# EmbersArc/SCpp

Hardware: AMD Instinct MI355X
Metric: converged SCvx trajectories/sec (RocketQuat, K=50) at 1/2/4/8 MI355X (higher is better)
Workload: dtype f64

## Files before the change

### scpp_amd/csrc/common.h

```cpp
#pragma once
#ifdef SCPP_HIP_EMU
#include "hip_emu.h"
#else
#include <hip/hip_runtime.h>
typedef double d4_t __attribute__((ext_vector_type(4)));
#endif
#include <cmath>
#include <cstdint>

namespace scpp
{

constexpr int WAVE = 64;

#ifdef SCPP_HIP_EMU
#define WAVE_SYNC() __syncthreads()
#else
#define WAVE_SYNC()                                            \
    do                                                         \
    {                                                          \
        __builtin_amdgcn_fence(__ATOMIC_ACQ_REL, "wavefront"); \
        __builtin_amdgcn_wave_barrier();                       \
    } while (0)
#endif

#ifdef SCPP_HIP_EMU
template <class T>
inline T *uniformPtr(T *p) { return p; }
inline int uniformInt(int v) { return v; }
#else
template <class T>
__device__ __forceinline__ T *uniformPtr(T *p)
{
    const unsigned long long v = reinterpret_cast<unsigned long long>(p);
    const unsigned lo = __builtin_amdgcn_readfirstlane(unsigned(v)), hi = __builtin_amdgcn_readfirstlane(unsigned(v >> 32));
    typedef __attribute__((address_space(1))) T *gptr_t;
    return (T *)(gptr_t)((unsigned long long)(hi) << 32 | lo);
}
__device__ __forceinline__ int uniformInt(int v) { return __builtin_amdgcn_readfirstlane(v); }
#endif

#ifdef SCPP_HIP_EMU
inline double fastRcp(double d) { return 1. / d; }
inline double fastRsqrt(double d) { return 1. / sqrt(d); }
#else
__device__ __forceinline__ double fastRcp(double d)
{
    double r = __builtin_amdgcn_rcp(d);
    double e = __builtin_fma(-d, r, 1.);
    r = __builtin_fma(r, e, r);
    e = __builtin_fma(-d, r, 1.);
    r = __builtin_fma(r, e, r);
    return r;
}
__device__ __forceinline__ double fastRsqrt(double d)
{
    double y = __builtin_amdgcn_rsq(d);
    double h = 0.5 * y, e = __builtin_fma(-d * y, h, 0.5);
    y = __builtin_fma(y, e, y);
    h = 0.5 * y;
    e = __builtin_fma(-d * y, h, 0.5);
    y = __builtin_fma(y, e, y);
// ... 208 lines not shown
```

### scpp_amd/csrc/ipm_kernel.h

```cpp
#pragma once
#include "common.h"
#include "cone_math.h"
#include "constraint_table.h"
#include <type_traits>
#include <utility>

namespace scpp
{
namespace ipm
{

#ifndef IPM_FAC_ALIGN
#define IPM_FAC_ALIGN 1
#endif
template <class P>
struct Lay : Derived<P>
{
    using D = Derived<P>;
    static constexpr int NX = P::NX, NU = P::NU, NXV = P::NXV, NUV = P::NUV, NS = D::NS, NL = D::NL, HS_N = D::HS_N;
    static constexpr int F_W = 0;
    static constexpr int F_DL = F_W + NV;
    static constexpr int F_DW = F_DL + 1;
    static constexpr int F_DDL = F_DW + NV;
    static constexpr int F_WBAR = F_DDL + 1;
// ... 161 lines not shown
    double feastol, abstol, reltol, gamma;
    int maxit;
    int use_mfma;
};

#ifdef SCPP_HIP_EMU
#define LDSP
#else
#define LDSP __attribute__((address_space(3)))
#endif
enum SegLdsSlot
{
    SL_LAM = 0,
    SL_NU,
    SL_NUB,
    NSEGLDS
};
struct Ctx
{
    LDSP double *segl;
    int K, lane;
    int pitch;
    int setup_v0;
    double *st;
    double *sg;
    double *dy;
    double *fac;
    double *sv;
    double *sx;
    double *gsave;
    const double *A, *B, *C, *S, *Z;
    const double *ip;
};

template <class P>
__host__ __device__ inline unsigned segLdsBytes(int K)
{
    return SegInLds<P>::value ? unsigned(NSEGLDS * Lay<P>::NL * recPitch(K) * 8) : 0u;
}

template <class F, int... Is>
__device__ inline void sforImpl(F &&f, std::integer_sequence<int, Is...>)
{
    (f(std::integral_constant<int, Is>{}), ...);
}
template <int N, class F>
// ... 311 lines not shown
```

### scpp_amd/csrc/ipm_solve.h

```cpp
#pragma once
#include "ipm_kernel.h"
#include "sweeps.h"
#include <type_traits>

namespace scpp
{
namespace ipm
{

#define IPM_BLOWN 1e30
#ifndef IPM_SPLIT_STEPS
#define IPM_SPLIT_STEPS 1
#endif
#ifndef IPM_FUSE_UPDATE
#define IPM_FUSE_UPDATE 1
#endif
#define IPM_NEG_GAP 1e-6
__device__ inline bool ipmGapBroken(double gap) { return fabs(gap) > IPM_BLOWN || gap < -IPM_NEG_GAP; }

struct Glob
{
    double sig, dsg, n1, sigbar;
    double ss, zs, s3, z3, sc3[3], zc3[3];
    double dsig, ddsg, dn1, dss, dzs, ds3, dz3, dsc3[3], dzc3[3];
    double seta, sw[3];
    double hsig, Hsd, Hdd, schur;
    double lamC[3], dsC[3], dzC[3];
};

struct KernelArgs
{
    int B, K;
    double *X, *U, *sigma;
    const double *A, *Bm, *C, *S, *Z;
    const double *ip;
    const double *uhat;
    double *ws;
    double *wtrx;
    int *active;
    int *converged, *sc_iters, *ipm_iters, *status;
    double *norm1_nu, *sum_delta, *delta_sigma;
    double nu_tol, delta_tol;
    int max_sc_iterations;
    int *warm;
    int do_sc_update;
    int setup_schedule;
    const int *dd_fresh;
    double *Xold, *Uold;
    Settings opt;
    double *dbg;
};

struct Rhs
{
    double s, ds, n1, rhs3;
};

__device__ inline double dLP(bool identity, double sv, double zv) { return identity ? 1. : zv / sv; }

template <class P>
__device__ inline void prepareFactor(const Ctx &c, bool identity, Glob &g)
{
    using L = Lay<P>;
    const int k = c.lane, K = c.K;
    if (k < K - 1 && identity)
    {
        const SV sg = makeSV(c.sg, (G_NFIELDS * L::NL), unsigned(k), c.pitch);
        const SV xs = makeSX(c.sx, L::XREC, K, unsigned(k));
#pragma unroll
// ... 1689 lines not shown
            inj_m = -1;
            if (sscanf(e, "%d:%lf:%lf:%lf", &inj_n, &inj_v[0], &inj_v[1], &inj_v[2]) != 4)
                inj_n = -1;
        }
    }
    const int call = inj_n >= 0 ? calls[lane & (LANES - 1)]++ : -1;
    if (inj_n >= 0 && (call == inj_n || call == inj_m))
    {
        pres = inj_v[0];
        dres = inj_v[1];
        gap = inj_v[2];
    }
}
#endif
struct ResAcc
{
    double gap, rx, ry, rz, xx, yy, zz, ss, rxs, sumnb;
};
struct PendingStep
{
    double om, sigmu, z3_old, dz3, dsig, alpha, alpha_d;
};
template <class P, int I0, int N, bool UPD>
__device__ inline void resSegChunk(const SV &sg, const SegLds &sl, const SV &dyz, const SV &xs, const SV &xsz, double z3, ResAcc &p, const PendingStep &u)
{
    using L = Lay<P>;
    double nu[N], nub[N], s1[N], z1[N], s2[N], z2[N], lam[N], S[N];
    ldf<N>(sg, G_S1 * L::NL + I0, s1);
    ldf<N>(sg, G_Z1 * L::NL + I0, z1);
    ldf<N>(sg, G_S2 * L::NL + I0, s2);
    ldf<N>(sg, G_Z2 * L::NL + I0, z2);
    ldl<P, SL_NU, I0, N>(sl, nu);
    ldl<P, SL_NUB, I0, N>(sl, nub);
    ldl<P, SL_LAM, I0, N>(sl, lam);
    ldf<N>(dyz, L::DY_S + I0, S);
    if constexpr (UPD)
    {
        double vl[N], bcl[N], p1[N], p2[N];
        ldf<N>(xs, L::X_VL + I0, vl);
        ldf<N>(xsz, L::X_BCL + I0, bcl);
        ldf<N>(sg, G_DS1 * L::NL + I0, p1);
        ldf<N>(sg, G_DS2 * L::NL + I0, p2);
        LOADS_ISSUED();
#pragma unroll
        for (int i = 0; i < N; i++)
        {
            const SegRhsRow r = segRhsRow<1>(nu[i], nub[i], s1[i], z1[i], s2[i], z2[i], lam[i], p1[i], p2[i], u.om, u.sigmu, u.z3_old, u.dz3);
// ... 14 lines not shown
        stf<N>(sg, G_S2 * L::NL + I0, s2);
        stf<N>(sg, G_Z2 * L::NL + I0, z2);
    }
    else
        LOADS_ISSUED();
#pragma unroll
    for (int i = 0; i < N; i++)
    {
        const double r1 = s1[i] - (nub[i] - nu[i]);
        const double r2 = s2[i] - (nub[i] + nu[i]);
        const double rnu = -lam[i] + z1[i] - z2[i];
        const double rnub = -z1[i] - z2[i] + z3;
        p.sumnb += nub[i];
        p.gap += s1[i] * z1[i] + s2[i] * z2[i];
        p.rz += r1 * r1 + r2 * r2;
        p.zz += z1[i] * z1[i] + z2[i] * z2[i];
        p.ss += s1[i] * s1[i] + s2[i] * s2[i];
        p.yy += lam[i] * lam[i];
        p.rx += rnu * rnu + rnub * rnub;
        p.xx += nu[i] * nu[i] + nub[i] * nub[i];
        p.rxs += S[i] * lam[i];
    }
}
template <class P, bool UPD>
PHASE_FN void phResiduals(const PRIV Ctx *cin, PRIV Glob *gp, PRIV Iter *ip_)
{
    EMU_PHASE(UPD ? "phResiduals<update>" : "phResiduals");
    using L = Lay<P>;
    constexpr int NX = P::NX, NU = P::NU;
    const Ctx c = uniformCtx(cin);
    const Views v = makeViews<P>(c);
    const int k = v.k;
    const SV &st = v.st, &stN = v.stN, &sg = v.sg, &sgP = v.sgP, &dy = v.dy, &dyP = v.dyP;
    const double *ip = c.ip;
    const unsigned fm = v.fm;
    PendingStep u{0., 0., 0., 0., 0., 0., 0.};
    if constexpr (UPD)
    {
        Glob g = loadPriv(gp);
        const double sigma_c = ip_->sigma_c;
        u.alpha = ip_->alpha;
        u.alpha_d = ip_->alpha_d;
        u.om = 1. - sigma_c;
        u.sigmu = sigma_c * double(ip_->mu);
        u.z3_old = g.z3;
        u.dz3 = g.dz3;
        u.dsig = g.dsig;
        const double alpha = u.alpha, alpha_d = u.alpha_d;
// ... 188 lines not shown
        {
            const bool fx = fm & (1u << j);
            const double r = -gw[j] + (fx ? 0. : acc[j]);
            rxw[j] = r;
            p.rx += fx ? 0. : r * r;
            p.xx += fx ? 0. : x0[j] * x0[j];
        }
        st[L::F_RXD] = rxd;
        stf<NV>(st, L::F_RXW, rxw);
        if (v.vsg)
            stf<L::NL>(sg, G_RY * L::NL, resv);
    }
    p.gap = waveSumDpp(p.gap);
    p.rx = waveSumDpp(p.rx);
    p.ry = waveSumDpp(p.ry);
    p.rz = waveSumDpp(p.rz);
    p.xx = waveSumDpp(p.xx);
    p.yy = waveSumDpp(p.yy);
    p.zz = waveSumDpp(p.zz);
    p.ss = waveSumDpp(p.ss);
    p.rxs = waveSumDpp(p.rxs);
    p.sumnb = waveSumDpp(p.sumnb);
    p_dl = waveSumDpp(p_dl);
    const Glob g = reloadPriv(gp);
    Iter it = reloadPriv(ip_);
    const double pres_before = it.pres;
    const double sas = g.sig - 0.001, sa3 = g.n1 - p.sumnb;
    const double sac[3] = {0.5 + 0.5 * g.dsg, 0.5 - 0.5 * g.dsg, g.sig - g.sigbar};
    it.rzs = g.ss - sas;
    it.rz3 = g.s3 - sa3;
    for (int i = 0; i < 3; i++)
        it.rzc[i] = g.sc3[i] - sac[i];
    it.rxs = it.w_t - g.zs - g.zc3[2] - p.rxs;
    it.rxds = it.w_trt - 0.5 * g.zc3[0] + 0.5 * g.zc3[1];
    it.rxn1 = it.w_vc - g.z3;
    double gap = p.gap + g.ss * g.zs + g.s3 * g.z3;
    double nrz = p.rz + it.rzs * it.rzs + it.rz3 * it.rz3;
    double nzz = p.zz + g.zs * g.zs + g.z3 * g.z3;
    double nss = p.ss + g.ss * g.ss + g.s3 * g.s3;
    for (int i = 0; i < 3; i++)
    {
        gap += g.sc3[i] * g.zc3[i];
        nrz += it.rzc[i] * it.rzc[i];
        nzz += g.zc3[i] * g.zc3[i];
        nss += g.sc3[i] * g.sc3[i];
    }
    const double nrx = p.rx + it.rxs * it.rxs + it.rxds * it.rxds + it.rxn1 * it.rxn1;
    const double nxx = p.xx + g.sig * g.sig + g.dsg * g.dsg + g.n1 * g.n1;
    it.gap = gap;
    it.mu = gap / it.D;
    it.pcost = it.w_t * g.sig + it.w_trt * g.dsg + it.w_vc * g.n1 + it.wtrx * p_dl;
    {
        const double nx_ = sqrt(nxx), ny_ = sqrt(p.yy), nz_ = sqrt(nzz), ns_ = sqrt(nss);
        const double d1 = it.resy0 + nx_ > 1. ? it.resy0 + nx_ : 1.;
        const double d2 = it.resz0 + nx_ + ns_ > 1. ? it.resz0 + nx_ + ns_ : 1.;
        const double pa = sqrt(p.ry) / d1, pb = sqrt(nrz) / d2;
        it.pres = pa > pb ? pa : pb;
        const double d3 = it.resx0 + ny_ + nz_ > 1. ? it.resx0 + ny_ + nz_ : 1.;
        it.dres = sqrt(nrx) / d3;
    }
#ifdef SCPP_HIP_EMU
    emuInjectResiduals(c.lane, it.pres, it.dres, it.gap);
#endif
    {
        const double apc = fabs(it.pcost) > 1e-300 ? fabs(it.pcost) : 1e-300;
        const bool broken = !(it.pres == it.pres) || !(it.dres == it.dres) || !(it.gap == it.gap) || fabs(it.pres) > 1e300 || fabs(it.dres) > 1e300 ||
                            ipmGapBroken(it.gap) || fabs(it.pcost) > IPM_BLOWN ||
                            (it.bk_valid != 0 && (it.pres > 500. * pres_before || it.gap < 0.));
        const bool inacc = !broken && it.pres < 1e-4 && it.dres < 1e-4 && (it.gap < 5e-5 || it.gap / apc < 5e-5);
        if (inacc)
        {
            if (v.vst)
            {
                double xw[NV + 1];
                ldf<NV + 1>(st, L::F_W, xw);
                stf<NV + 1>(st, L::F_WBK, xw);
            }
            it.bk_sig = g.sig;
            it.bk_dsg = g.dsg;
            it.bk_n1 = g.n1;
            it.bk_valid = 1;
        }
        PUT_BEGIN();
        PUT(ip_, it, rzs);
        PUT(ip_, it, rz3);
        PUT(ip_, it, rzc);
        PUT(ip_, it, rxs);
        PUT(ip_, it, rxds);
        PUT(ip_, it, rxn1);
        PUT(ip_, it, gap);
        PUT(ip_, it, mu);
        PUT(ip_, it, pcost);
        PUT(ip_, it, pres);
        PUT(ip_, it, dres);
        if (inacc)
        {
            PUT(ip_, it, bk_sig);
            PUT(ip_, it, bk_dsg);
            PUT(ip_, it, bk_n1);
            PUT(ip_, it, bk_valid);
        }
        PUT_END();
    }
}

template <class P>
PHASE_FN void phScalings(const PRIV Ctx *cin, PRIV Glob *gp, PRIV Iter *ip_)
{
    EMU_PHASE("phScalings");
    using L = Lay<P>;
    const Ctx c = uniformCtx(cin);
    const Views v = makeViews<P>(c);
    const SV &st = v.st;
    const unsigned act = v.act;
    const bool scvx = scvxMode(c.ip);
    const SV stz = padView(v.st, scvx);
    Glob g = loadPriv(gp);
    int bad = 0;
    if (v.vst)
    {
        forEachCone<P>([&](auto ci) {
            constexpr int C = decltype(ci)::value;
            if (act & (1u << C))
                bad |= coneScaling<P, L::coneOff(C), L::coneDim(C)>(st, C, stz);
        });
    }
// ... 723 lines not shown
        for (int i = 0; i < 10; i++)
            sh.prof[i] = 0.;
#endif
    const int K = a.K, lane = threadIdx.x, k = lane;
    Ctx c;
    c.K = K;
    c.lane = lane;
    double *ws = a.ws + size_t(inst) * workspaceDoubles<P>(K);
    c.sx = ws;
    c.st = ws + size_t(K) * L::XREC;
    c.pitch = recPitch(K);
    c.sg = c.st + size_t(c.pitch) * L::STREC;
    c.dy = c.sg + size_t(c.pitch) * (G_NFIELDS * L::NL);
    c.fac = ws + facOffset<P>(K);
    c.sv = c.fac + size_t(K) * L::FACREC;
    c.gsave = c.sv + size_t(K) * SVREC;
    c.A = a.A + size_t(inst) * (K - 1) * NX * NX;
    c.B = a.Bm + size_t(inst) * (K - 1) * NX * NU;
    c.C = a.C + size_t(inst) * (K - 1) * NX * NU;
    c.S = a.S + size_t(inst) * (K - 1) * NX;
    c.Z = a.Z + size_t(inst) * (K - 1) * NX;
    c.ip = a.ip + size_t(inst) * IP_N;
    c.setup_v0 = a.setup_schedule == 0;
    EMU_PHASE("solve: outside the phases");
    EMU_TRAFFIC_REGION("exchange [K][XREC]", c.sx, size_t(K) * L::XREC * 8, 8, size_t(L::XREC) * 8);
    EMU_TRAFFIC_REGION("stage [STREC][K]", c.st, size_t(c.pitch) * L::STREC * 8, size_t(c.pitch) * 8, 0);
    EMU_TRAFFIC_REGION("segment [G_NFIELDS*NL][K]", c.sg, size_t(c.pitch) * (G_NFIELDS * L::NL) * 8, size_t(c.pitch) * 8, 0);
    EMU_TRAFFIC_REGION("dd copy [DYNREC][K]", c.dy, size_t(c.pitch) * L::DYNREC * 8, size_t(c.pitch) * 8, 0);
    EMU_TRAFFIC_REGION("factor [K][FACREC]", c.fac, size_t(K) * L::FACREC * 8, 8, size_t(L::FACREC) * 8);
    EMU_TRAFFIC_REGION("saved columns [K][SVREC]", c.sv, size_t(K) * SVREC * 8, 8, size_t(SVREC) * 8);
    EMU_TRAFFIC_REGION("dd A [K-1][NX][NX]", c.A, size_t(K - 1) * NX * NX * 8, 8, size_t(NX) * NX * 8);
    EMU_TRAFFIC_REGION("dd B [K-1][NX][NU]", c.B, size_t(K - 1) * NX * NU * 8, 8, size_t(NX) * NU * 8);
    EMU_TRAFFIC_REGION("dd C [K-1][NX][NU]", c.C, size_t(K - 1) * NX * NU * 8, 8, size_t(NX) * NU * 8);
#ifdef SCPP_HIP_EMU
    static double seg_lds[NSEGLDS * 16 * 64];
    c.segl = seg_lds;
#else
    extern __shared__ __attribute__((aligned(16))) double seg_lds[];
    c.segl = (LDSP double *)seg_lds;
#endif
    const Settings opt = a.opt;

    __shared__ Glob g;
    __shared__ Iter it;
    __shared__ Ctx cshared;
    PRIV Glob *gp = (PRIV Glob *)&g;
// ... 45 lines not shown
            const RhsSpec sp = specSingle();
            fwdSweepAny<P>(cs, sp);
            bwdSweepAny<P>(cs, sp);
        }
        phInitDualFinish<P>(cs, gp, itp);
    }
    solveDataNorms<P>(cs, gp, itp, dd_same);
    phSegLdsCopy<P, true>(cs);
    PROF_T(tp1);
    PROF_ADD(0, tp0, tp1);

    status = -1;
    iter = 0;
    use_backup = false;
    it.bk_valid = 0;
    it.bad = 0;
    bool inacc_ok = false, bk_prev = false;
    double pres_prev = 0.;
    for (iter = 0;; iter++)
    {
        PROF_T(tr0);
#if IPM_FUSE_UPDATE
        if (iter == 0)
            phResiduals<P, false>(cs, gp, itp);
        else
            phResiduals<P, true>(cs, gp, itp);
#else
        phResiduals<P, false>(cs, gp, itp);
#endif
        PROF_T(tr1);
        PROF_ADD(1, tr0, tr1);
        {
            const double pres = it.pres, dres = it.dres, gap = it.gap;
            const double apc = fabs(it.pcost) > 1e-300 ? fabs(it.pcost) : 1e-300;
            const double relgap = gap / apc;
#ifdef SCPP_HIP_EMU
            if (c.lane == 0 && getenv("SCPP_EMU_DEBUG"))
                printf("[emu] iter %d pres %.3e dres %.3e gap %.3e pcost %.9e | last step: alpha %.3e alpha_d %.3e sigma_c %.3e\n", iter, pres, dres, gap, double(it.pcost),
                       double(it.alpha), double(it.alpha_d), double(it.sigma_c));
#endif
            const bool nonfinite = !(pres == pres) || !(dres == dres) || !(gap == gap) || fabs(pres) > 1e300 || fabs(dres) > 1e300 || fabs(gap) > 1e300 ||
                                   fabs(it.pcost) > IPM_BLOWN || ipmGapBroken(gap);
            if (nonfinite || (bk_prev && iter > 0 && (pres > 500. * pres_prev || gap < 0.)))
            {
                status = bk_prev ? 0 : -2;
                use_backup = bk_prev;
                break;
            }
            pres_prev = pres;
            bk_prev = it.bk_valid != 0;
            if (pres < opt.feastol && dres < opt.feastol && (gap < opt.abstol || relgap < opt.reltol))
// ... 188 lines not shown
```

### scpp_amd/csrc/ipm_split.h

```cpp
#pragma once
#include "ipm_solve.h"

namespace scpp
{
namespace ipm
{

#ifndef IPM_SPLIT_WAVES
#define IPM_SPLIT_WAVES 3
#endif

enum SplitPc
{
    PC_START = 0,
    PC_INIT_F = 1,
    PC_MAIN_F = 2,
    PC_NORMS = 3,
    PC_HEAD = 4,
    PC_END = 5,
    PC_DONE = 6
};
constexpr int RS_GLOB = 0, RS_ITER = RS_GLOB + int(sizeof(Glob) / 8), RS_LOC = RS_ITER + int(sizeof(Iter) / 8);
enum SplitLocal
{
// ... 17 lines not shown
    using L = Lay<P>;
    constexpr int NX = P::NX, NU = P::NU;
    const int K = a.K;
    Ctx c;
    c.K = K;
    c.lane = lane;
    double *ws = a.ws + size_t(inst) * workspaceDoubles<P>(K);
    c.sx = ws;
    c.st = ws + size_t(K) * L::XREC;
    c.pitch = recPitch(K);
    c.sg = c.st + size_t(c.pitch) * L::STREC;
    c.dy = c.sg + size_t(c.pitch) * (G_NFIELDS * L::NL);
    c.fac = ws + facOffset<P>(K);
    c.sv = c.fac + size_t(K) * L::FACREC;
    c.gsave = c.sv + size_t(K) * SVREC;
    c.A = a.A + size_t(inst) * (K - 1) * NX * NX;
    c.B = a.Bm + size_t(inst) * (K - 1) * NX * NU;
    c.C = a.C + size_t(inst) * (K - 1) * NX * NU;
    c.S = a.S + size_t(inst) * (K - 1) * NX;
    c.Z = a.Z + size_t(inst) * (K - 1) * NX;
    c.ip = a.ip + size_t(inst) * IP_N;
    c.segl = nullptr;
    c.setup_v0 = a.setup_schedule == 0;
    return c;
}

template <class T>
__device__ inline void saveUniform(double *dst, const PRIV T *src, int lane)
{
    const PRIV double *s = (const PRIV double *)src;
    for (int i = lane; i < int(sizeof(T) / 8); i += WAVE)
        dst[i] = s[i];
}
template <class T>
__device__ inline void loadUniform(PRIV T *dst, const double *src, int lane)
{
    PRIV double *d = (PRIV double *)dst;
    for (int i = lane; i < int(sizeof(T) / 8); i += WAVE)
        d[i] = src[i];
}

template <class P>
__global__ void __launch_bounds__(WAVE) ipm_split_finalize_kernel(KernelArgs a)
{
    const int inst = blockIdx.x * WAVE + threadIdx.x;
    if (inst >= a.B)
// ... 141 lines not shown
                fwdSweepAny<W>(cs, sp);
                bwdSweepAny<W>(cs, sp);
            }
            phInitDualFinish<W>(cs, gp, itp);
            pc = PC_NORMS;
        }
        else if (pc == PC_NORMS)
        {
            solveDataNorms<W>(cs, gp, itp, 0);
            status = -1;
            iter = 0;
            use_backup = false;
            it.bk_valid = 0;
            it.bad = 0;
            inacc_ok = false;
            bk_prev = false;
            pres_prev = 0.;
            pc = PC_HEAD;
        }
        else if (pc == PC_HEAD)
        {
#if IPM_FUSE_UPDATE
            if (iter == 0)
                phResiduals<W, false>(cs, gp, itp);
            else
                phResiduals<W, true>(cs, gp, itp);
#else
            phResiduals<W, false>(cs, gp, itp);
#endif
            {
                const double pres = it.pres, dres = it.dres, gap = it.gap;
                const double apc = fabs(it.pcost) > 1e-300 ? fabs(it.pcost) : 1e-300;
                const double relgap = gap / apc;
                const bool nonfinite = !(pres == pres) || !(dres == dres) || !(gap == gap) || fabs(pres) > 1e300 || fabs(dres) > 1e300 || fabs(gap) > 1e300 ||
                                   fabs(it.pcost) > IPM_BLOWN || ipmGapBroken(gap);
                if (nonfinite || (bk_prev && iter > 0 && (pres > 500. * pres_prev || gap < 0.)))
                {
                    status = bk_prev ? 0 : -2;
                    use_backup = bk_prev;
                    pc = PC_END;
                    continue;
                }
                pres_prev = pres;
                bk_prev = it.bk_valid != 0;
                if (pres < opt.feastol && dres < opt.feastol && (gap < opt.abstol || relgap < opt.reltol))
                {
                    status = 0;
                    pc = PC_END;
                    continue;
                }
                inacc_ok = pres < 1e-4 && dres < 1e-4 && (gap < 5e-5 || relgap < 5e-5);
// ... 171 lines not shown
```

### scpp_amd/csrc/scpp_hip.cpp

```cpp
#include "../../include/scpp_hip.h"

#include <algorithm>
#include <cmath>
#include <utility>
#include <cstdio>
#include <cstdlib>
#include <cstring>
#include <mutex>
#include <new>
#include <tuple>
#include <type_traits>
#include <vector>

#include "common.h"
#include "discretize_kernel.h"
#include "ipm_solve.h"
#include "ipm_split.h"
#include "model_rocketquat.h"
#include "sc_kernels.h"
#include "scvx_kernels.h"
#include "scvx_persistent.h"
#include "mpc_kernel.h"
#include "mpc_setup.h"

// ... 71 lines not shown
    bool sc_ready = false, par_from_ip = false;
    bool sc_warm = false;
    int sc_persistent_min = 3072;
    int mode = SCPP_MODE_FOH | SCPP_MODE_VT;
    struct Span
    {
        hipEvent_t a, b;
        int kind;
        long long inst;
    };
    std::vector<Span> spans;
    std::vector<hipEvent_t> pool;
    scpp_timing timing{};
    hipEvent_t ev_base = nullptr;
    int last_active = 0;
    long long stream_rounds = 0;
    int stream_pools = 0;
    int stream_engine = SCPP_STREAM_ENGINE_DEFAULT;
    double *persist_shares = nullptr;
    unsigned long long stream_ticks[4] = {0, 0, 0, 0};
    int ipm_schedule = SCPP_IPM_SCHEDULE_DEFAULT;
    int ipm_split_pairs = 0;
    int disc_schedule = DISC_STAGE_SCHEDULE;
    int setup_schedule = IPM_SETUP_SCHEDULE;
    int disc_steps = 5;
};

namespace
{

struct DeviceGuard
{
    int prev = -1;
    bool switched = false;
    explicit DeviceGuard(const scpp_hip_ctx *c)
    {
        if (!c)
            return;
        if (hipGetDevice(&prev) == hipSuccess && prev != c->device)
            switched = hipSetDevice(c->device) == hipSuccess;
    }
    ~DeviceGuard()
    {
        if (switched)
            (void)hipSetDevice(prev);
    }
// ... 225 lines not shown
    a.A = c->A + f * seg * nx * nx;
    a.Bm = c->Bm + f * seg * nx * nu;
    a.C = c->C + f * seg * nx * nu;
    a.S = c->S + f * seg * nx;
    a.Z = c->Z + f * seg * nx;
    a.ip = c->ip + f * ipm::IP_N;
    a.uhat = c->uhat + f * K * 3;
    a.ws = c->ws + f * c->ws_per;
    a.wtrx = c->wtrx + f;
    a.active = (do_sc_update || masked) ? c->active + f : nullptr;
    a.converged = c->converged + f;
    a.sc_iters = c->sc_iters + f;
    a.ipm_iters = c->ipm_iters + f;
    a.status = c->status + f;
    a.norm1_nu = c->norm1_nu + f;
    a.sum_delta = c->sum_delta + f;
    a.delta_sigma = c->delta_sigma + f;
    a.nu_tol = c->sc.nu_tol;
    a.delta_tol = c->sc.delta_tol;
    a.max_sc_iterations = c->sc.max_iterations;
    a.warm = c->ipm_warm + f;
    a.do_sc_update = do_sc_update;
    a.setup_schedule = c->setup_schedule;
    a.dd_fresh = (snapshot && c->ipm_schedule == SCPP_IPM_RESIDENT) ? c->vx_needs_disc + f : nullptr;
    a.Xold = snapshot ? c->vx_Xold + f * K * nx : nullptr;
    a.Uold = snapshot ? c->vx_Uold + f * K * nu : nullptr;
    a.opt.feastol = c->socp.feastol;
    a.opt.abstol = c->socp.abstol;
    a.opt.reltol = c->socp.reltol;
    a.opt.gamma = 0.99;
    a.opt.maxit = c->socp.maxit;
    a.opt.use_mfma = c->socp.use_mfma;
    a.dbg = c->dbg + f * 32;
    return a;
}
int launchIpm(scpp_hip_ctx *c, int do_sc_update, long long ninst, bool masked, Range r, unsigned lds_pad = 0, bool snapshot = false)
{
    const ipm::KernelArgs a = ipmArgs(c, do_sc_update, masked, r, snapshot);
    const bool timed = spanBegin(c, 1, ninst, r.stream);
    const bool zoh = !(c->mode & SCPP_MODE_FOH);
    (void)withPlugin(c->model, [&](auto pl) {
        using PL = decltype(pl);
        using T = typename PL::Table;
        const unsigned grid = unsigned(r.count);
        if constexpr (PL::SPLIT_SCHEDULE)
        {
// ... 174 lines not shown
            if (d >= 0)
                (void)hipSetDevice(d);
        }
    } restore{prev_device == device_id ? -1 : prev_device};
    if (int rc = tileSelfTest(device_id))
        return rc;
    scpp_hip_ctx *c = new (std::nothrow) scpp_hip_ctx;
    if (!c)
        return SCPP_E_HIP;
    c->device = device_id;
    c->model = model_id;
    c->K = K;
    c->Bmax = batch_max;
    c->B = 0;
    if (const char *e = std::getenv("SCPP_IPM_SCHEDULE"))
        if (std::atoi(e) >= SCPP_IPM_RESIDENT && std::atoi(e) <= SCPP_IPM_SPLIT)
            c->ipm_schedule = std::atoi(e);
    if (const char *e = std::getenv("SCPP_DISC_SCHEDULE"))
        if (std::atoi(e) == 0)
            c->disc_schedule = 0;
    if (const char *e = std::getenv("SCPP_SETUP_SCHEDULE"))
        if (std::atoi(e) == 0)
            c->setup_schedule = 0;
    if (const char *e = std::getenv("SCPP_STREAM_ENGINE"))
        if (std::atoi(e) == SCPP_STREAM_POOLS || std::atoi(e) == SCPP_STREAM_PERSISTENT)
            c->stream_engine = std::atoi(e);
    if (const char *e = std::getenv("SCPP_SC_PERSISTENT_MIN"))
        if (std::atoi(e) > 0)
            c->sc_persistent_min = std::atoi(e);
    if (const char *e = std::getenv("SCPP_IPM_SPLIT_PAIRS"))
        if (std::atoi(e) > 0)
            c->ipm_split_pairs = std::atoi(e);
    (void)withPlugin(model_id, [&](auto pl) {
        using PL = decltype(pl);
        c->nx = PL::Model::NX;
        c->nu = PL::Model::NU;
        c->np = PL::Model::NP;
        c->ws_per = ipm::workspaceDoubles<typename PL::Table>(K);
        return 0;
    });
    if (hipStreamCreate(&c->stream) != hipSuccess)
    {
        delete c;
        return SCPP_E_HIP;
    }
    const size_t B = size_t(batch_max), nx = c->nx, nu = c->nu;
// ... 1561 lines not shown
```

### scpp_amd/csrc/sweeps.h

```cpp
#pragma once
#include "tile_engine.h"

namespace scpp
{
namespace ipm
{

#ifndef IPM_PRIO_FACTOR
#define IPM_PRIO_FACTOR 1
#endif
#ifndef IPM_PRIO_SUBST
#define IPM_PRIO_SUBST 2
#endif
#if defined(SCPP_HIP_EMU)
#define SET_PRIO(p)
#else
#define SET_PRIO(p) __builtin_amdgcn_s_setprio(p)
#endif
#ifndef SWEEP_PREFETCH
#define SWEEP_PREFETCH 2
#endif
#ifndef SWEEPS_INLINE
#define SWEEP_FN static __device__ __attribute__((noinline, disable_tail_calls))
#else
#define SWEEP_FN __device__ inline __attribute__((always_inline))
#endif

__device__ inline LDSP double *uniformLds(LDSP double *p)
{
#ifdef SCPP_HIP_EMU
    return p;
#else
    return (LDSP double *)(unsigned long long)(unsigned)__builtin_amdgcn_readfirstlane((unsigned)(unsigned long long)p);
#endif
}
__device__ inline Ctx uniformCtx(const LDSP Ctx *cin)
{
    Ctx c;
    c.segl = uniformLds(cin->segl);
    c.K = uniformInt(cin->K);
    c.lane = threadIdx.x;
    c.pitch = uniformInt(cin->pitch);
    c.setup_v0 = uniformInt(cin->setup_v0);
    c.st = uniformPtr(cin->st);
    c.sg = uniformPtr(cin->sg);
    c.dy = uniformPtr(cin->dy);
    c.fac = uniformPtr(cin->fac);
    c.sv = uniformPtr(cin->sv);
    c.sx = uniformPtr(cin->sx);
    c.gsave = uniformPtr(cin->gsave);
    c.A = uniformPtr(cin->A);
    c.B = uniformPtr(cin->B);
    c.C = uniformPtr(cin->C);
    c.S = uniformPtr(cin->S);
    c.Z = uniformPtr(cin->Z);
    c.ip = uniformPtr(cin->ip);
    return c;
}
#ifndef IPM_FAC_LD_AUX
#define IPM_FAC_LD_AUX IPM_LD_AUX
#endif
#ifndef IPM_FAC_ST_AUX
#define IPM_FAC_ST_AUX 2
#endif
#ifndef IPM_DD_LD_AUX
#define IPM_DD_LD_AUX IPM_LD_AUX
// ... 1064 lines not shown
```

Before: 6422.

## Add software-pipelined residual pass with row-ahead loads and early wave reductions

Adds a new default residual phase that walks the dynamics rows with compile-time recursion and loads row I+1's coefficients while computing row I. It also reduces several accumulators early, broadcasting them as scalars via readfirstlane, and factors the termination logic into a shared helper. The old path stays available through an env var. The aim is to hide global-load latency in the residual computation, at the cost of more live registers and a possible occupancy drop.

Result: no change. 6461 (median of 6 runs) (+0.6%).

```diff
diff --git a/scpp_amd/csrc/common.h b/scpp_amd/csrc/common.h
--- a/scpp_amd/csrc/common.h
+++ b/scpp_amd/csrc/common.h
@@ -28,6 +28,7 @@
 template <class T>
 inline T *uniformPtr(T *p) { return p; }
 inline int uniformInt(int v) { return v; }
+inline double uniformDouble(double v) { return v; }
 #else
 template <class T>
 __device__ __forceinline__ T *uniformPtr(T *p)
@@ -38,6 +39,12 @@
     return (T *)(gptr_t)((unsigned long long)(hi) << 32 | lo);
 }
 __device__ __forceinline__ int uniformInt(int v) { return __builtin_amdgcn_readfirstlane(v); }
+__device__ __forceinline__ double uniformDouble(double v)
+{
+    const unsigned long long b = __builtin_bit_cast(unsigned long long, v);
+    const unsigned lo = __builtin_amdgcn_readfirstlane(unsigned(b)), hi = __builtin_amdgcn_readfirstlane(unsigned(b >> 32));
+    return __builtin_bit_cast(double, (static_cast<unsigned long long>(hi) << 32) | lo);
+}
 #endif
 
 #ifdef SCPP_HIP_EMU
diff --git a/scpp_amd/csrc/ipm_kernel.h b/scpp_amd/csrc/ipm_kernel.h
--- a/scpp_amd/csrc/ipm_kernel.h
+++ b/scpp_amd/csrc/ipm_kernel.h
@@ -207,6 +207,7 @@
     int K, lane;
     int pitch;
     int setup_v0;
+    int res_v0;
     double *st;
     double *sg;
     double *dy;
diff --git a/scpp_amd/csrc/ipm_solve.h b/scpp_amd/csrc/ipm_solve.h
--- a/scpp_amd/csrc/ipm_solve.h
+++ b/scpp_amd/csrc/ipm_solve.h
@@ -45,6 +45,7 @@
     int *warm;
     int do_sc_update;
     int setup_schedule;
+    int residual_schedule;
     const int *dd_fresh;
     double *Xold, *Uold;
     Settings opt;
@@ -1780,7 +1781,7 @@
     double om, sigmu, z3_old, dz3, dsig, alpha, alpha_d;
 };
 template <class P, int I0, int N, bool UPD>
-__device__ inline void resSegChunk(const SV &sg, const SegLds &sl, const SV &dyz, const SV &xs, const SV &xsz, double z3, ResAcc &p, const PendingStep &u)
+__device__ __forceinline__ void resSegChunk(const SV &sg, const SegLds &sl, const SV &dyz, const SV &xs, const SV &xsz, double z3, ResAcc &p, const PendingStep &u)
 {
     using L = Lay<P>;
     double nu[N], nub[N], s1[N], z1[N], s2[N], z2[N], lam[N], S[N];
@@ -1841,8 +1842,94 @@
         p.rxs += S[i] * lam[i];
     }
 }
+template <class P>
+__device__ __forceinline__ void resTermination(const Ctx &c, const Views &v, PRIV Glob *gp, PRIV Iter *ip_, const ResAcc &p, double p_dl)
+{
+    using L = Lay<P>;
+    const SV &st = v.st;
+    const Glob g = reloadPriv(gp);
+    Iter it = reloadPriv(ip_);
+    const double pres_before = it.pres;
+    const double sas = g.sig - 0.001, sa3 = g.n1 - p.sumnb;
+    const double sac[3] = {0.5 + 0.5 * g.dsg, 0.5 - 0.5 * g.dsg, g.sig - g.sigbar};
+    it.rzs = g.ss - sas;
+    it.rz3 = g.s3 - sa3;
+    for (int i = 0; i < 3; i++)
+        it.rzc[i] = g.sc3[i] - sac[i];
+    it.rxs = it.w_t - g.zs - g.zc3[2] - p.rxs;
+    it.rxds = it.w_trt - 0.5 * g.zc3[0] + 0.5 * g.zc3[1];
+    it.rxn1 = it.w_vc - g.z3;
+    double gap = p.gap + g.ss * g.zs + g.s3 * g.z3;
+    double nrz = p.rz + it.rzs * it.rzs + it.rz3 * it.rz3;
+    double nzz = p.zz + g.zs * g.zs + g.z3 * g.z3;
+    double nss = p.ss + g.ss * g.ss + g.s3 * g.s3;
+    for (int i = 0; i < 3; i++)
+    {
+        gap += g.sc3[i] * g.zc3[i];
+        nrz += it.rzc[i] * it.rzc[i];
+        nzz += g.zc3[i] * g.zc3[i];
+        nss += g.sc3[i] * g.sc3[i];
+    }
+    const double nrx = p.rx + it.rxs * it.rxs + it.rxds * it.rxds + it.rxn1 * it.rxn1;
+    const double nxx = p.xx + g.sig * g.sig + g.dsg * g.dsg + g.n1 * g.n1;
+    it.gap = gap;
+    it.mu = gap / it.D;
+    it.pcost = it.w_t * g.sig + it.w_trt * g.dsg + it.w_vc * g.n1 + it.wtrx * p_dl;
+    {
+        const double nx_ = sqrt(nxx), ny_ = sqrt(p.yy), nz_ = sqrt(nzz), ns_ = sqrt(nss);
+        const double d1 = it.resy0 + nx_ > 1. ? it.resy0 + nx_ : 1.;
+        const double d2 = it.resz0 + nx_ + ns_ > 1. ? it.resz0 + nx_ + ns_ : 1.;
+        const double pa = sqrt(p.ry) / d1, pb = sqrt(nrz) / d2;
+        it.pres = pa > pb ? pa : pb;
+        const double d3 = it.resx0 + ny_ + nz_ > 1. ? it.resx0 + ny_ + nz_ : 1.;
+        it.dres = sqrt(nrx) / d3;
+    }
+#ifdef SCPP_HIP_EMU
+    emuInjectResiduals(c.lane, it.pres, it.dres, it.gap);
+#endif
+    {
+        const double apc = fabs(it.pcost) > 1e-300 ? fabs(it.pcost) : 1e-300;
+        const bool broken = !(it.pres == it.pres) || !(it.dres == it.dres) || !(it.gap == it.gap) || fabs(it.pres) > 1e300 || fabs(it.dres) > 1e300 ||
+                            ipmGapBroken(it.gap) || fabs(it.pcost) > IPM_BLOWN ||
+                            (it.bk_valid != 0 && (it.pres > 500. * pres_before || it.gap < 0.));
+        const bool inacc = !broken && it.pres < 1e-4 && it.dres < 1e-4 && (it.gap < 5e-5 || it.gap / apc < 5e-5);
+        if (inacc)
+        {
+            if (v.vst)
+            {
+                double xw[NV + 1];
+                ldf<NV + 1>(st, L::F_W, xw);
+                stf<NV + 1>(st, L::F_WBK, xw);
+            }
+            it.bk_sig = g.sig;
+            it.bk_dsg = g.dsg;
+            it.bk_n1 = g.n1;
+            it.bk_valid = 1;
+        }
+        PUT_BEGIN();
+        PUT(ip_, it, rzs);
+        PUT(ip_, it, rz3);
+        PUT(ip_, it, rzc);
+        PUT(ip_, it, rxs);
+        PUT(ip_, it, rxds);
+        PUT(ip_, it, rxn1);
+        PUT(ip_, it, gap);
+        PUT(ip_, it, mu);
+        PUT(ip_, it, pcost);
+        PUT(ip_, it, pres);
+        PUT(ip_, it, dres);
+        if (inacc)
+        {
+            PUT(ip_, it, bk_sig);
+            PUT(ip_, it, bk_dsg);
+            PUT(ip_, it, bk_n1);
+            PUT(ip_, it, bk_valid);
+        }
+        PUT_END();
+    }
+}
 template <class P, bool UPD>
-PHASE_FN void phResiduals(const PRIV Ctx *cin, PRIV Glob *gp, PRIV Iter *ip_)
+PHASE_FN void phResidualsV0(const PRIV Ctx *cin, PRIV Glob *gp, PRIV Iter *ip_)
 {
     EMU_PHASE(UPD ? "phResiduals<update>" : "phResiduals");
     using L = Lay<P>;
@@ -2077,86 +2164,343 @@
     p.rxs = waveSumDpp(p.rxs);
     p.sumnb = waveSumDpp(p.sumnb);
     p_dl = waveSumDpp(p_dl);
-    const Glob g = reloadPriv(gp);
-    Iter it = reloadPriv(ip_);
-    const double pres_before = it.pres;
-    const double sas = g.sig - 0.001, sa3 = g.n1 - p.sumnb;
-    const double sac[3] = {0.5 + 0.5 * g.dsg, 0.5 - 0.5 * g.dsg, g.sig - g.sigbar};
-    it.rzs = g.ss - sas;
-    it.rz3 = g.s3 - sa3;
-    for (int i = 0; i < 3; i++)
-        it.rzc[i] = g.sc3[i] - sac[i];
-    it.rxs = it.w_t - g.zs - g.zc3[2] - p.rxs;
-    it.rxds = it.w_trt - 0.5 * g.zc3[0] + 0.5 * g.zc3[1];
-    it.rxn1 = it.w_vc - g.z3;
-    double gap = p.gap + g.ss * g.zs + g.s3 * g.z3;
-    double nrz = p.rz + it.rzs * it.rzs + it.rz3 * it.rz3;
-    double nzz = p.zz + g.zs * g.zs + g.z3 * g.z3;
-    double nss = p.ss + g.ss * g.ss + g.s3 * g.s3;
-    for (int i = 0; i < 3; i++)
-    {
-        gap += g.sc3[i] * g.zc3[i];
-        nrz += it.rzc[i] * it.rzc[i];
-        nzz += g.zc3[i] * g.zc3[i];
-        nss += g.sc3[i] * g.sc3[i];
-    }
-    const double nrx = p.rx + it.rxs * it.rxs + it.rxds * it.rxds + it.rxn1 * it.rxn1;
-    const double nxx = p.xx + g.sig * g.sig + g.dsg * g.dsg + g.n1 * g.n1;
-    it.gap = gap;
-    it.mu = gap / it.D;
-    it.pcost = it.w_t * g.sig + it.w_trt * g.dsg + it.w_vc * g.n1 + it.wtrx * p_dl;
-    {
-        const double nx_ = sqrt(nxx), ny_ = sqrt(p.yy), nz_ = sqrt(nzz), ns_ = sqrt(nss);
-        const double d1 = it.resy0 + nx_ > 1. ? it.resy0 + nx_ : 1.;
-        const double d2 = it.resz0 + nx_ + ns_ > 1. ? it.resz0 + nx_ + ns_ : 1.;
-        const double pa = sqrt(p.ry) / d1, pb = sqrt(nrz) / d2;
-        it.pres = pa > pb ? pa : pb;
-        const double d3 = it.resx0 + ny_ + nz_ > 1. ? it.resx0 + ny_ + nz_ : 1.;
-        it.dres = sqrt(nrx) / d3;
-    }
-#ifdef SCPP_HIP_EMU
-    emuInjectResiduals(c.lane, it.pres, it.dres, it.gap);
-#endif
-    {
-        const double apc = fabs(it.pcost) > 1e-300 ? fabs(it.pcost) : 1e-300;
-        const bool broken = !(it.pres == it.pres) || !(it.dres == it.dres) || !(it.gap == it.gap) || fabs(it.pres) > 1e300 || fabs(it.dres) > 1e300 ||
-                            ipmGapBroken(it.gap) || fabs(it.pcost) > IPM_BLOWN ||
-                            (it.bk_valid != 0 && (it.pres > 500. * pres_before || it.gap < 0.));
-        const bool inacc = !broken && it.pres < 1e-4 && it.dres < 1e-4 && (it.gap < 5e-5 || it.gap / apc < 5e-5);
-        if (inacc)
-        {
-            if (v.vst)
-            {
-                double xw[NV + 1];
-                ldf<NV + 1>(st, L::F_W, xw);
-                stf<NV + 1>(st, L::F_WBK, xw);
-            }
-            it.bk_sig = g.sig;
-            it.bk_dsg = g.dsg;
-            it.bk_n1 = g.n1;
-            it.bk_valid = 1;
+    resTermination<P>(c, v, gp, ip_, p, p_dl);
+}
+
+#ifndef IPM_RESIDUAL_SCHEDULE
+#define IPM_RESIDUAL_SCHEDULE 1
+#endif
+#if IPM_RESIDUAL_SCHEDULE
+#ifndef IPM_RES_ROW_AHEAD
+#define IPM_RES_ROW_AHEAD 2
+#endif
+template <class P>
+struct ResRowA
+{
+    double ra[P::NXV];
+};
+template <class P>
+struct ResRowB
+{
+    double rb[P::NUV], rc[P::NUV];
+#if defined(SCPP_HIP_EMU) || RES_PREVLANE_MEMORY
+    double rcp[P::NUV];
+#endif
+    double xn, s, z, lam, lamP, nu;
+};
+template <class P, int I>
+__device__ __forceinline__ ResRowA<P> resLoadRowA(const SV &dy)
+{
+    using L = Lay<P>;
+    ResRowA<P> r;
+    sfor<P::NXV>([&](auto jt) { r.ra[decltype(jt)::value] = dy[L::DY_A + I * P::NX + P::XMAP[decltype(jt)::value]]; });
+    return r;
+}
+template <class P, int I>
+__device__ __forceinline__ ResRowB<P> resLoadRowB(const SV &dy, const SV &dyP, const SV &dyz, const SV &stN, const SegLds &sl, const SegLds &slP)
+{
+    using L = Lay<P>;
+    constexpr int xi = L::XINV.v[I];
+    ResRowB<P> r;
+    sfor<P::NUV>([&](auto jt) { r.rb[decltype(jt)::value] = dy[L::DY_B + I * P::NU + P::UMAP[decltype(jt)::value]]; });
+    sfor<P::NUV>([&](auto jt) { r.rc[decltype(jt)::value] = dy[L::DY_C + I * P::NU + P::UMAP[decltype(jt)::value]]; });
+#if defined(SCPP_HIP_EMU) || RES_PREVLANE_MEMORY
+    sfor<P::NUV>([&](auto jt) { r.rcp[decltype(jt)::value] = dyP[L::DY_C + I * P::NU + P::UMAP[decltype(jt)::value]]; });
+#else
+    (void)dyP;
+#endif
+    r.xn = xi >= 0 ? double(stN[L::F_W + (xi >= 0 ? xi : 0)]) : 0.;
+    r.s = dyz[L::DY_S + I];
+    r.z = dy[L::DY_Z + I];
+    if constexpr (!SegInLds<P>::value)
+    {
+        r.lam = segLdsGet<P, SL_LAM>(sl, I);
+        r.lamP = segLdsGet<P, SL_LAM>(slP, I);
+        r.nu = segLdsGet<P, SL_NU>(sl, I);
+    }
+    return r;
+}
+template <class P, int I>
+__device__ __forceinline__ double resRow(const ResRowA<P> &a, const ResRowB<P> &b, const SegLds &sl, const SegLds &slP, double mk, double mp, double g_sig,
+                                         const double (&x0)[NV], const double (&u1)[P::NUV], double (&acc)[NV])
+{
+    constexpr int NXV = P::NXV, NUV = P::NUV, xi = Lay<P>::XINV.v[I];
+    double rcp[NUV];
+#if defined(SCPP_HIP_EMU) || RES_PREVLANE_MEMORY
+    sfor<NUV>([&](auto jt) { rcp[decltype(jt)::value] = b.rcp[decltype(jt)::value]; });
+#else
+    sfor<NUV>([&](auto jt) { rcp[decltype(jt)::value] = prevLane(b.rc[decltype(jt)::value]); });
+#endif
+    const double lam = SegInLds<P>::value ? segLdsGet<P, SL_LAM>(sl, I) : b.lam, lamP = SegInLds<P>::value ? segLdsGet<P, SL_LAM>(slP, I) : b.lamP;
+    const double nu = SegInLds<P>::value ? segLdsGet<P, SL_NU>(sl, I) : b.nu;
+    const double l = mk * lam, lp = mp * lamP;
+    double rr = b.xn - b.s * g_sig - nu - b.z;
+#pragma unroll
+    for (int j = 0; j < NXV; j++)
+    {
+        acc[j] -= a.ra[j] * l;
+        rr -= a.ra[j] * x0[j];
+    }
+#pragma unroll
+    for (int j = 0; j < NUV; j++)
+    {
+        acc[NXV + j] -= b.rb[j] * l + rcp[j] * lp;
+        rr -= b.rb[j] * x0[NXV + j] + b.rc[j] * u1[j];
+    }
+    if constexpr (xi >= 0)
+        acc[xi] += lp;
+#ifndef SCPP_HIP_EMU
+#pragma unroll
+    for (int j = 0; j < NV; j++)
+        asm volatile("" : "+v"(acc[j]));
+#endif
+    return rr;
+}
+template <class P, int I>
+__device__ __forceinline__ void resRows(const ResRowA<P> &a, const ResRowB<P> &b0, const SV &dy, const SV &dyP, const SV &dyz, const SV &stN, const SegLds &sl,
+                                        const SegLds &slP, const SV &sgRy, double mk, double mp, double g_sig, bool vsg, const double (&x0)[NV],
+                                        const double (&u1)[P::NUV], double (&acc)[NV], double &p_ry)
+{
+    constexpr int NL = Lay<P>::NL;
+    ResRowB<P> b = b0;
+    if constexpr (IPM_RES_ROW_AHEAD < 2)
+        b = resLoadRowB<P, I>(dy, dyP, dyz, stN, sl, slP);
+    ResRowA<P> an;
+    ResRowB<P> bn;
+    if constexpr (I + 1 < NL)
+    {
+        an = resLoadRowA<P, I + 1>(dy);
+        if constexpr (IPM_RES_ROW_AHEAD >= 2)
+            bn = resLoadRowB<P, I + 1>(dy, dyP, dyz, stN, sl, slP);
+    }
+    LOADS_ISSUED();
+    const double rr = resRow<P, I>(a, b, sl, slP, mk, mp, g_sig, x0, u1, acc);
+    sgRy[G_RY * NL + I] = rr;
+    p_ry += vsg ? rr * rr : 0.;
+    if constexpr (I + 1 < NL)
+        resRows<P, I + 1>(an, bn, dy, dyP, dyz, stN, sl, slP, sgRy, mk, mp, g_sig, vsg, x0, u1, acc, p_ry);
+}
+template <class P, bool UPD>
+PHASE_FN void phResiduals(const PRIV Ctx *cin, PRIV Glob *gp, PRIV Iter *ip_)
+{
+    EMU_PHASE(UPD ? "phResiduals<update>" : "phResiduals");
+    using L = Lay<P>;
+    constexpr int NX = P::NX, NU = P::NU;
+    const Ctx c = uniformCtx(cin);
+    const Views v = makeViews<P>(c);
+    const int k = v.k;
+    const SV &st = v.st, &stN = v.stN, &sg = v.sg, &sgP = v.sgP, &dy = v.dy, &dyP = v.dyP;
+    const double *ip = c.ip;
+    const unsigned fm = v.fm;
+    PendingStep u{0., 0., 0., 0., 0., 0., 0.};
+    if constexpr (UPD)
+    {
+        Glob g = loadPriv(gp);
+        const double sigma_c = ip_->sigma_c;
+        u.alpha = ip_->alpha;
+        u.alpha_d = ip_->alpha_d;
+        u.om = 1. - sigma_c;
+        u.sigmu = sigma_c * double(ip_->mu);
+        u.z3_old = g.z3;
+        u.dz3 = g.dz3;
+        u.dsig = g.dsig;
+        const double alpha = u.alpha, alpha_d = u.alpha_d;
+        g.sig += alpha * g.dsig;
+        g.dsg += alpha * g.ddsg;
+        g.n1 += alpha * g.dn1;
+        g.ss += alpha * g.dss;
+        g.zs += alpha_d * g.dzs;
+        g.s3 += alpha * g.ds3;
+        g.z3 += alpha_d * g.dz3;
+        for (int i = 0; i < 3; i++)
+        {
+            g.sc3[i] += alpha * g.dsc3[i];
+            g.zc3[i] += alpha_d * g.dzc3[i];
         }
         PUT_BEGIN();
-        PUT(ip_, it, rzs);
-        PUT(ip_, it, rz3);
-        PUT(ip_, it, rzc);
-        PUT(ip_, it, rxs);
-        PUT(ip_, it, rxds);
-        PUT(ip_, it, rxn1);
-        PUT(ip_, it, gap);
-        PUT(ip_, it, mu);
-        PUT(ip_, it, pcost);
-        PUT(ip_, it, pres);
-        PUT(ip_, it, dres);
-        if (inacc)
-        {
-            PUT(ip_, it, bk_sig);
-            PUT(ip_, it, bk_dsg);
-            PUT(ip_, it, bk_n1);
-            PUT(ip_, it, bk_valid);
-        }
+        PUT(gp, g, sig);
+        PUT(gp, g, dsg);
+        PUT(gp, g, n1);
+        PUT(gp, g, ss);
+        PUT(gp, g, zs);
+        PUT(gp, g, s3);
+        PUT(gp, g, z3);
+        PUT(gp, g, sc3);
+        PUT(gp, g, zc3);
         PUT_END();
     }
+    const double g_z3 = gp->z3, g_sig = gp->sig, it_wtrx = ip_->wtrx;
+    const bool scvx = scvxMode(ip);
+    const SV stz = padView(v.st, scvx);
+    const SV dyz = padView(v.dy, scvx);
+    const SegLds sl = makeSegLds<P>(c, v.vsg ? k : 0), slP = makeSegLds<P>(c, (k > 0 && k < v.K) ? k - 1 : 0);
+    ResAcc p;
+    p.gap = p.rx = p.ry = p.rz = p.xx = p.yy = p.zz = p.ss = p.rxs = p.sumnb = 0.;
+    double p_dl = 0.;
+    if (v.vsg)
+    {
+        const SV xsz = padView(v.xs, scvx);
+        forSegChunks<P, chunkFor<P>(IPM_RES_CHUNK, IPM_RES_CHUNK_W)>(
+            [&](auto i0, auto n) { resSegChunk<P, decltype(i0)::value, decltype(n)::value, UPD>(sg, sl, dyz, v.xs, xsz, g_z3, p, u); });
+    }
+    double x0[NV], gw[NV], gdl = 0., dl = 0.;
+    if (v.vst)
+    {
+        {
+            double wbar[NV], uh[3], sa[L::NS], sv[L::NS], zv[L::NS];
+            ldf<NV>(st, L::F_W, x0);
+            ldf<NV>(st, L::F_WBAR, wbar);
+            ldf<3>(st, L::F_UHAT, uh);
+            dl = st[L::F_DL];
+            if constexpr (UPD)
+            {
+                constexpr int H0 = (L::NS + 1) / 2, H1 = L::NS - H0;
+                {
+                    double dw[NV];
+                    ldf<NV>(st, L::F_DW, dw);
+                    const double ddl = st[L::F_DDL];
+                    LOADS_ISSUED();
+#pragma unroll
+                    for (int j = 0; j < NV; j++)
+                        x0[j] = x0[j] + ((fm & (1u << j)) ? 0. : u.alpha * dw[j]);
+                    dl = dl + u.alpha * ddl;
+                }
+                ldPad<L::NS, P::NXV>(st, stz, L::F_S, sv);
+                {
+                    double d[H0];
+                    ldPadPart<P::NXV, 0, H0>(st, stz, L::F_DS, d);
+                    LOADS_ISSUED();
+#pragma unroll
+                    for (int i = 0; i < H0; i++)
+                        sv[i] = sv[i] + u.alpha * d[i];
+                }
+                {
+                    double d[H1];
+                    ldPadPart<P::NXV, H0, H1>(st, stz, L::F_DS, d);
+                    LOADS_ISSUED();
+#pragma unroll
+                    for (int i = 0; i < H1; i++)
+                        sv[H0 + i] = sv[H0 + i] + u.alpha * d[i];
+                }
+                ldPad<L::NS, P::NXV>(st, stz, L::F_Z, zv);
+                stf<NV>(st, L::F_W, x0);
+                st[L::F_DL] = dl;
+                stPad<L::NS, P::NXV>(st, stz, L::F_S, sv);
+            }
+            else
+            {
+                ldPad<L::NS, P::NXV>(st, stz, L::F_S, sv);
+                LOADS_ISSUED();
+            }
+            saff<P>(ip, v.act, x0, dl, wbar, uh, sa);
+#pragma unroll
+            for (int i = 0; i < L::NS; i++)
+            {
+                sa[i] = sv[i] - sa[i];
+                p.rz += sa[i] * sa[i];
+                p.ss += sv[i] * sv[i];
+            }
+            if constexpr (UPD)
+            {
+                constexpr int H0 = (L::NS + 1) / 2, H1 = L::NS - H0;
+                stPad<L::NS, P::NXV>(st, stz, L::F_RZ, sa);
+                {
+                    double d[H0];
+                    ldPadPart<P::NXV, 0, H0>(st, stz, L::F_DZ, d);
+                    LOADS_ISSUED();
+#pragma unroll
+                    for (int i = 0; i < H0; i++)
+                        zv[i] = zv[i] + u.alpha_d * d[i];
+                }
+                {
+                    double d[H1];
+                    ldPadPart<P::NXV, H0, H1>(st, stz, L::F_DZ, d);
+                    LOADS_ISSUED();
+#pragma unroll
+                    for (int i = 0; i < H1; i++)
+                        zv[H0 + i] = zv[H0 + i] + u.alpha_d * d[i];
+                }
+                stPad<L::NS, P::NXV>(st, stz, L::F_Z, zv);
+            }
+            else
+            {
+                ldPad<L::NS, P::NXV>(st, stz, L::F_Z, zv);
+                LOADS_ISSUED();
+                stPad<L::NS, P::NXV>(st, stz, L::F_RZ, sa);
+            }
+#pragma unroll
+            for (int i = 0; i < L::NS; i++)
+            {
+                p.gap += sv[i] * zv[i];
+                p.zz += zv[i] * zv[i];
+            }
+            LTmul<P>(ip, fm, zv, uh, gw, &gdl);
+        }
+    }
+    p.gap = uniformDouble(waveSumDpp(p.gap));
+    p.rz = uniformDouble(waveSumDpp(p.rz));
+    p.yy = uniformDouble(waveSumDpp(p.yy));
+    p.zz = uniformDouble(waveSumDpp(p.zz));
+    p.ss = uniformDouble(waveSumDpp(p.ss));
+    p.rxs = uniformDouble(waveSumDpp(p.rxs));
+    p.sumnb = uniformDouble(waveSumDpp(p.sumnb));
+    double p_ry = 0.;
+    if constexpr (UPD)
+    {
+#ifndef SCPP_HIP_EMU
+        __builtin_amdgcn_s_waitcnt(0);
+#endif
+        WAVE_SYNC();
+    }
+    if (v.vst)
+    {
+        const double rxd = (ip[IP_SCVX] != 0.) ? 0. : it_wtrx - gdl;
+        constexpr int NXV = P::NXV, NUV = P::NUV;
+        double acc[NV], u1[NUV];
+#pragma unroll
+        for (int j = 0; j < NV; j++)
+            acc[j] = 0.;
+        ldf<NUV>(stN, L::F_W + NXV, u1);
+        const double mk = v.vsg ? 1. : 0., mp = k > 0 ? 1. : 0.;
+        {
+            const ResRowA<P> a0 = resLoadRowA<P, 0>(dy);
+            ResRowB<P> b0;
+            if constexpr (IPM_RES_ROW_AHEAD >= 2)
+                b0 = resLoadRowB<P, 0>(dy, dyP, dyz, stN, sl, slP);
+            resRows<P, 0>(a0, b0, dy, dyP, dyz, stN, sl, slP, padView(sg, !v.vsg), mk, mp, g_sig, v.vsg, x0, u1, acc, p_ry);
+        }
+        p.rx += rxd * rxd;
+        p.xx += dl * dl;
+        p_dl += dl;
+        double rxw[NV];
+#pragma unroll
+        for (int j = 0; j < NV; j++)
+        {
+            const bool fx = fm & (1u << j);
+            const double r = -gw[j] + (fx ? 0. : acc[j]);
+            rxw[j] = r;
+            p.rx += fx ? 0. : r * r;
+            p.xx += fx ? 0. : x0[j] * x0[j];
+        }
+        st[L::F_RXD] = rxd;
+        stf<NV>(st, L::F_RXW, rxw);
+    }
+    p.rx = waveSumDpp(p.rx);
+    p.ry = waveSumDpp(p_ry);
+    p.xx = waveSumDpp(p.xx);
+    p_dl = waveSumDpp(p_dl);
+    resTermination<P>(c, v, gp, ip_, p, p_dl);
+}
+#endif
+template <class P, bool UPD>
+__device__ inline void residualPass(const PRIV Ctx *cin, PRIV Glob *gp, PRIV Iter *ip_)
+{
+    if (!IPM_RESIDUAL_SCHEDULE || uniformInt(cin->res_v0) != 0)
+        phResidualsV0<P, UPD>(cin, gp, ip_);
+#if IPM_RESIDUAL_SCHEDULE
+    else
+        phResiduals<P, UPD>(cin, gp, ip_);
+#endif
 }
 
 template <class P>
@@ -2926,6 +3270,7 @@
     c.Z = a.Z + size_t(inst) * (K - 1) * NX;
     c.ip = a.ip + size_t(inst) * IP_N;
     c.setup_v0 = a.setup_schedule == 0;
+    c.res_v0 = a.residual_schedule == 0;
     EMU_PHASE("solve: outside the phases");
     EMU_TRAFFIC_REGION("exchange [K][XREC]", c.sx, size_t(K) * L::XREC * 8, 8, size_t(L::XREC) * 8);
     EMU_TRAFFIC_REGION("stage [STREC][K]", c.st, size_t(c.pitch) * L::STREC * 8, size_t(c.pitch) * 8, 0);
@@ -3017,11 +3362,11 @@
         PROF_T(tr0);
 #if IPM_FUSE_UPDATE
         if (iter == 0)
-            phResiduals<P, false>(cs, gp, itp);
+            residualPass<P, false>(cs, gp, itp);
         else
-            phResiduals<P, true>(cs, gp, itp);
+            residualPass<P, true>(cs, gp, itp);
 #else
-        phResiduals<P, false>(cs, gp, itp);
+        residualPass<P, false>(cs, gp, itp);
 #endif
         PROF_T(tr1);
         PROF_ADD(1, tr0, tr1);
diff --git a/scpp_amd/csrc/ipm_split.h b/scpp_amd/csrc/ipm_split.h
--- a/scpp_amd/csrc/ipm_split.h
+++ b/scpp_amd/csrc/ipm_split.h
@@ -63,6 +63,7 @@
     c.ip = a.ip + size_t(inst) * IP_N;
     c.segl = nullptr;
     c.setup_v0 = a.setup_schedule == 0;
+    c.res_v0 = a.residual_schedule == 0;
     return c;
 }
 
@@ -250,11 +251,11 @@
         {
 #if IPM_FUSE_UPDATE
             if (iter == 0)
-                phResiduals<W, false>(cs, gp, itp);
+                residualPass<W, false>(cs, gp, itp);
             else
-                phResiduals<W, true>(cs, gp, itp);
+                residualPass<W, true>(cs, gp, itp);
 #else
-            phResiduals<W, false>(cs, gp, itp);
+            residualPass<W, false>(cs, gp, itp);
 #endif
             {
                 const double pres = it.pres, dres = it.dres, gap = it.gap;
diff --git a/scpp_amd/csrc/scpp_hip.cpp b/scpp_amd/csrc/scpp_hip.cpp
--- a/scpp_amd/csrc/scpp_hip.cpp
+++ b/scpp_amd/csrc/scpp_hip.cpp
@@ -117,6 +117,7 @@
     int ipm_schedule = SCPP_IPM_SCHEDULE_DEFAULT;
     int ipm_split_pairs = 0;
     int disc_schedule = DISC_STAGE_SCHEDULE;
+    int residual_schedule = IPM_RESIDUAL_SCHEDULE;
     int setup_schedule = IPM_SETUP_SCHEDULE;
     int disc_steps = 5;
 };
@@ -388,6 +389,7 @@
     a.warm = c->ipm_warm + f;
     a.do_sc_update = do_sc_update;
     a.setup_schedule = c->setup_schedule;
+    a.residual_schedule = c->residual_schedule;
     a.dd_fresh = (snapshot && c->ipm_schedule == SCPP_IPM_RESIDENT) ? c->vx_needs_disc + f : nullptr;
     a.Xold = snapshot ? c->vx_Xold + f * K * nx : nullptr;
     a.Uold = snapshot ? c->vx_Uold + f * K * nu : nullptr;
@@ -608,6 +610,9 @@
     if (const char *e = std::getenv("SCPP_SETUP_SCHEDULE"))
         if (std::atoi(e) == 0)
             c->setup_schedule = 0;
+    if (const char *e = std::getenv("SCPP_RESIDUAL_SCHEDULE"))
+        if (std::atoi(e) == 0)
+            c->residual_schedule = 0;
     if (const char *e = std::getenv("SCPP_STREAM_ENGINE"))
         if (std::atoi(e) == SCPP_STREAM_POOLS || std::atoi(e) == SCPP_STREAM_PERSISTENT)
             c->stream_engine = std::atoi(e);
diff --git a/scpp_amd/csrc/sweeps.h b/scpp_amd/csrc/sweeps.h
--- a/scpp_amd/csrc/sweeps.h
+++ b/scpp_amd/csrc/sweeps.h
@@ -42,6 +42,7 @@
     c.lane = threadIdx.x;
     c.pitch = uniformInt(cin->pitch);
     c.setup_v0 = uniformInt(cin->setup_v0);
+    c.res_v0 = uniformInt(cin->res_v0);
     c.st = uniformPtr(cin->st);
     c.sg = uniformPtr(cin->sg);
     c.dy = uniformPtr(cin->dy);
```
